# zhongzisha/multi_frame_super_resolution

Measured on AMD Instinct MI355X. Metric: Mpix/s end-to-end (N-frame burst -> x2 SR), higher is better.
Workload: dtype f32

## Files before the change

### include/mfsr.h

```cpp
#ifndef MFSR_H
#define MFSR_H

#include <stddef.h>
#include <stdint.h>

#ifdef __cplusplus
extern "C" {
#endif

#define MFSR_VERSION 100
#define MFSR_MAX_FUSE_GROUP 4
#define MFSR_MAX_BURST_FUSE 16

typedef void* mfsr_stream_t;

typedef struct { float x, y; } mfsr_float2;
typedef struct { float x, y, z; } mfsr_float3;
typedef struct { float x, y, z, w; } mfsr_float4;

typedef struct {
    const void* ptr;
    int32_t pitch;
    int32_t width;
    int32_t height;
// ... 330 lines not shown
    float Dth, Dtr, kDetail, kDenoise, kStretch, kShrink;
    float weightThreshold;
    int32_t applyGamma;
    int32_t fused;
    int32_t pairFrames;
    int32_t asyncFuse;
    int32_t preAlign;
    float preAlignMaxAngle;
    int32_t uploadRing;
    int32_t maskErode;
    int32_t rawPacking;
} mfsr_config;

typedef struct mfsr_burst mfsr_burst;

int mfsr_config_default(mfsr_config* cfg, int width, int height, int frames, int scale, int mono);
size_t mfsr_burst_workspace_bytes(const mfsr_config* cfg);
size_t mfsr_burst_accumulator_bytes(const mfsr_config* cfg);
int mfsr_burst_create(mfsr_burst** out, const mfsr_config* cfg, void* workspace, size_t workspaceBytes);
void mfsr_burst_destroy(mfsr_burst* b);

int mfsr_window_check(const mfsr_config* cfg, int x0, int y0, int w, int h);
int mfsr_burst_set_window(mfsr_burst* b, int x0, int y0, int w, int h);
int mfsr_burst_get_window(const mfsr_burst* b, int* x0, int* y0, int* w, int* h);
int mfsr_burst_set_reference(mfsr_burst* b, const uint16_t* rawRef, mfsr_stream_t stream);
int mfsr_burst_set_reference_rows(mfsr_burst* b, const uint16_t* rawRef, int hrRow0, int hrRow1, mfsr_stream_t stream);
int mfsr_burst_add_frame(mfsr_burst* b, const uint16_t* raw, int isReference, mfsr_float3* imgOut,
                         mfsr_float3* totalWeights, mfsr_stream_t stream);
int mfsr_burst_begin(mfsr_burst* b, mfsr_float3* imgOut, mfsr_float3* totalWeights, mfsr_stream_t stream);
int mfsr_burst_flush(mfsr_burst* b, mfsr_stream_t stream);
int mfsr_burst_hold_fuse(mfsr_burst* b, int enable);
int mfsr_burst_fuse_stats(const mfsr_burst* b, int* burstLaunches, int* groupsFused);
int mfsr_set_burst_fuse(int enable);
int mfsr_burst_finish(mfsr_burst* b, const mfsr_float3* imgOut, const mfsr_float3* totalWeights, mfsr_float3* outImg,
                      uint16_t* out16, mfsr_stream_t stream);
int mfsr_burst_finish_rows(mfsr_burst* b, const mfsr_float3* imgOut, const mfsr_float3* totalWeights,
                           mfsr_float3* outImg, uint16_t* out16, int row0, int rows, mfsr_stream_t stream);
int mfsr_burst_set_reference_host(mfsr_burst* b, const uint16_t* hostRaw, mfsr_stream_t stream);
int mfsr_burst_add_frame_host(mfsr_burst* b, const uint16_t* hostRaw, int isReference, mfsr_float3* imgOut,
                              mfsr_float3* totalWeights, mfsr_stream_t stream);
int mfsr_burst_prefetch_host(mfsr_burst* b, const uint16_t* const* hostRaws, int nFrames, mfsr_stream_t stream);
int mfsr_burst_finish_host(mfsr_burst* b, const mfsr_float3* imgOut, const mfsr_float3* totalWeights, uint16_t* out16Dev,
                           uint16_t* out16Host, mfsr_stream_t stream);
int mfsr_burst_host_sync(mfsr_burst* b);
int mfsr_burst_set_host_row_bytes(mfsr_burst* b, int rowBytes);
int mfsr_burst_field_dims(const mfsr_burst* b, int* flowW, int* flowH, int* maskW, int* maskH);
int mfsr_burst_align_frame(mfsr_burst* b, const uint16_t* raw, int isReference, mfsr_float2* flowOut, int flowPitch,
                           mfsr_float4* maskOut, int maskPitch, mfsr_stream_t stream);
int mfsr_burst_align_frames(mfsr_burst* b, int nFrames, const uint16_t* const* raws, const int* isReference,
                            mfsr_float2* const* flowOut, int flowPitch, mfsr_float4* const* maskOut, int maskPitch,
                            mfsr_stream_t stream);
int mfsr_burst_group_size(const mfsr_config* cfg);
int mfsr_burst_fuse_rows(mfsr_burst* b, int nFrames, const uint16_t* const* raws, const mfsr_float2* const* flows, int flowPitch,
                         const mfsr_float4* const* masks, int maskPitch, mfsr_float3* imgOut, mfsr_float3* totalWeights,
                         int accumulatorsUndefined, int rowBegin, int rowEnd, mfsr_stream_t stream);

typedef struct {
    int32_t rowBegin, rowEnd;
    int32_t flowRow0, flowRows;
    int32_t maskRow0, maskRows;
    int32_t rawRow0, rawRows;
    float maxFlowY;
    int32_t reserved[3];
} mfsr_stripe_plan;
int mfsr_dist_stripe_plan(const mfsr_config* cfg, int worldSize, int rank, int rawHalo, mfsr_stripe_plan* out);
int mfsr_checkFlowBound(const mfsr_float2* flow, int pitch, int width, int rows, float bound, int* flag, mfsr_stream_t stream);
// ... 243 lines not shown
```

### multi_frame_super_resolution_amd/csrc/accumulate_common.hpp

```cpp
#pragma once
#include <type_traits>
#include "common.hpp"

struct Levels3 {
    float white[3], black[3];
};

static inline Levels3 make_levels(mfsr_float3 white, mfsr_float3 black)
{
    Levels3 l;
    l.white[0] = white.x;
    l.white[1] = white.y;
    l.white[2] = white.z;
    l.black[0] = black.x;
    l.black[1] = black.y;
    l.black[2] = black.z;
    return l;
}

template <bool FAST>
__device__ __forceinline__ float tap_weight(int px, int py, float kx, float ky, float kz)
{
    float w = (float)(px * px) * kx + (float)(2 * px * py) * kz + (float)(py * py) * ky;
    if (FAST) {
        const float t = w * -0.72134752044448170368f;
        w = __builtin_amdgcn_exp2f(t);
    } else {
        w = expf(-0.5f * w);
    }
    if (!finitef(w)) w = (px * py == 0) ? 1.0f : 0.0f;
    return w;
}

__device__ __forceinline__ void tap_accumulate(float raw, float w, int color, const float4& cert4, const Levels3& lv,
                                               pix3& pixel, pix3& totalWeight)
// ... 154 lines not shown
        taps(std::false_type{});
    if (sums) {
#pragma unroll
        for (int ch = 0; ch < 3; ch++) {
            const float v = __builtin_fmaf(sumS[ch], wm * invWhite[ch], -(lv.black[ch] * invWhite[ch]) * sumW[ch]);
            if (ch == 0) pixel.x += v;
            if (ch == 1) pixel.y += v;
            if (ch == 2) pixel.z += v;
        }
        totalWeight.x += sumW[0];
        totalWeight.y += sumW[1];
        totalWeight.z += sumW[2];
    }
    (void)outW;
    (void)outH;
}

template <int GEOM, bool FAST, bool SUMS = false>
__device__ __forceinline__ void accumulate_pixel_generic(int x, int y, const uint16_t* __restrict__ dataIn,
                                                         pix3* __restrict__ imgOut, pix3* __restrict__ totalWeights,
                                                         const float4* __restrict__ certaintyMask,
                                                         const mfsr_tex2d& kernelParam, const mfsr_tex2d& shifts,
                                                         const Levels3& lv, int dimX, int dimY, int scale, int strideOut,
                                                         int strideMask, int cfa, int accX0 = 0, int accY0 = 0)
{
    pix3 pixel = row_ptr(imgOut, strideOut, y - accY0)[x - accX0];
    pix3 totalWeight = row_ptr(totalWeights, strideOut, y - accY0)[x - accX0];
    accumulate_pixel_core<GEOM, FAST, SUMS>(x, y, dataIn, certaintyMask, kernelParam, shifts, lv, dimX, dimY, scale, strideMask,
                                      cfa, pixel, totalWeight);
    row_ptr(imgOut, strideOut, y - accY0)[x - accX0] = pixel;
    row_ptr(totalWeights, strideOut, y - accY0)[x - accX0] = totalWeight;
}

struct HrWindow {
    int x0, y0, x1, y1;
    int rel;
};

struct MarginRects {
    int x0[4], y0[4], w[4];
    int start[5];
    int accX0, accY0;
};

inline MarginRects margin_rects(int hrW, int hrH, int M, const HrWindow& w)
{
    const int r[4][4] = {{1, 1, hrW - 1, M}, {1, hrH - M, hrW - 1, hrH - 1}, {1, M, M, hrH - M}, {hrW - M, M, hrW - 1, hrH - M}};
    MarginRects m{};
    m.start[0] = 0;
    for (int i = 0; i < 4; i++) {
        const int x0 = r[i][0] > w.x0 ? r[i][0] : w.x0, x1 = r[i][2] < w.x1 ? r[i][2] : w.x1;
        const int y0 = r[i][1] > w.y0 ? r[i][1] : w.y0, y1 = r[i][3] < w.y1 ? r[i][3] : w.y1;
        const int cw = x1 > x0 ? x1 - x0 : 0, ch = y1 > y0 ? y1 - y0 : 0;
        m.x0[i] = x0;
        m.y0[i] = y0;
        m.w[i] = cw > 0 ? cw : 1;
        m.start[i + 1] = m.start[i] + cw * ch;
    }
    m.accX0 = w.x0;
    m.accY0 = w.y0;
    return m;
}

__device__ __forceinline__ bool margin_rect_pixel(const MarginRects& m, int idx, int& x, int& y)
{
    if (idx >= m.start[4]) return false;
// ... 7 lines not shown
```

### multi_frame_super_resolution_amd/csrc/accumulate_fast.hip

```cpp
#include <cstdlib>

#include "accumulate_common.hpp"
#include <type_traits>

namespace {

template <int CFA>
struct Cfa {
    static constexpr int col(int yp, int xp) { return (CFA >> (2 * ((yp << 1) | xp))) & 3; }
    static constexpr int pos_of(int c)
    {
        int n = 0, p = -1;
        for (int a = 0; a < 4; a++)
            if (((CFA >> (2 * a)) & 3) == c) {
                n++;
                p = a;
            }
        return n == 1 ? p : -1;
    }
    static constexpr int count(int c)
    {
        int n = 0;
        for (int a = 0; a < 4; a++)
            if (((CFA >> (2 * a)) & 3) == c) n++;
// ... 234 lines not shown
        C[jt][2] = selm(mbx, P_(jt, 3), W_(jt, 4));
    }
    strip_pixel_sites<K, CFA>(C, s, mby, nby, mP, mQ, lv, accP, accW);
}

__device__ __forceinline__ void tap_pair_sums(const float (&w)[13], float (&P)[3][4])
{
    auto W_ = [&](int jt, int it) { const int n = jt * 5 + it; return w[n <= 12 ? n : 24 - n]; };
#pragma unroll
    for (int r = 0; r < 3; r++)
#pragma unroll
        for (int i = 0; i < 4; i++) P[r][i] = W_(r, i) + W_(r, i + 1);
}

template <int K, int CFA, int EP = 0, typename MaskF>
__device__ __forceinline__ void strip_pixel(int X, int Y, int sx, int sy, float kx, float ky, float kz,
                                             const uint16_t* __restrict__ raw, int dimX, MaskF mval,
                                             const StripLevels& lv, float* accP, float* accW)
{
    float w[13];
    tap_weights13(kx, ky, kz, w);
    auto rawf = [&](int x0, int y0, float (&s)[3][3]) {
        const uint16_t* r = raw + (size_t)y0 * dimX + x0;
#pragma unroll
        for (int j = 0; j < 3; j++)
#pragma unroll
            for (int i = 0; i < 3; i++) s[j][i] = (float)r[j * dimX + i];
    };
    strip_pixel_w<K, CFA, EP>(X, Y, sx, sy, w, rawf, mval, lv, accP, accW);
}

#define STRIP_MARGIN 16

template <int SCALE, bool WIN = false>
__global__ void __launch_bounds__(256)
    k_accumulateMargin(const uint16_t* __restrict__ raw, pix3* __restrict__ imgOut, pix3* __restrict__ totalWeights,
                       const float4* __restrict__ certaintyMask, mfsr_tex2d kernelParam, mfsr_tex2d shifts, Levels3 glv,
                       int dimX, int dimY, int strideOut, int strideMask, int cfaPacked, int rowBegin, int rowEnd, MarginRects mr)
{
    constexpr int scale = SCALE;
    if constexpr (WIN) {
        int x, y;
        if (!margin_rect_pixel(mr, blockIdx.x * blockDim.x + threadIdx.x, x, y)) return;
        accumulate_pixel_generic<GEOM_FULL, true, true>(x, y, raw, imgOut, totalWeights, certaintyMask, kernelParam, shifts,
                                                                   glv, dimX, dimY, scale, strideOut, strideMask, cfaPacked,
                                                                   mr.accX0, mr.accY0);
        return;
    }
    const int hrW = scale * dimX, hrH = scale * dimY, M = STRIP_MARGIN;
    const int rowLen = hrW - 2;
    const int nTop = (M - 1) * rowLen;
    const int nBot = (M - 1) * rowLen;
    const int sideLen = 2 * (M - 1);
    const int nSide = (hrH - 2 * M) * sideLen;
    const int idx = blockIdx.x * blockDim.x + threadIdx.x;
    int x, y;
    if (idx < nTop) {
        y = 1 + idx / rowLen;
        x = 1 + idx % rowLen;
    } else if (idx < nTop + nBot) {
        const int r = idx - nTop;
        y = hrH - M + r / rowLen;
        x = 1 + r % rowLen;
    } else if (idx < nTop + nBot + nSide) {
        const int r = idx - nTop - nBot;
        y = M + r / sideLen;
        const int c = r % sideLen;
        x = c < M - 1 ? 1 + c : hrW - M + (c - (M - 1));
    } else {
        return;
    }
    if (y < rowBegin || y >= rowEnd) return;
    accumulate_pixel_generic<GEOM_FULL, true, true>(x, y, raw, imgOut, totalWeights, certaintyMask, kernelParam, shifts, glv, dimX,
                                              dimY, scale, strideOut, strideMask, cfaPacked);
}

struct TileFrame {
    const uint16_t* raw;
    const float4* mask;
    mfsr_tex2d shifts;
};
template <int NF>
struct TileFrames {
    TileFrame f[NF];
};

template <int NF, int SCALE, bool WIN = false>
__global__ void __launch_bounds__(64 * NF)
    k_accumulateMarginN(TileFrames<NF> fr, pix3* __restrict__ imgOut, pix3* __restrict__ totalWeights, mfsr_tex2d kernelParam,
                        Levels3 glv, int dimX, int dimY, int strideOut, int strideMask, int cfaPacked, int rowBegin, int rowEnd,
                        MarginRects mr)
{
    constexpr int scale = SCALE;
    __shared__ float sSum[NF][6][64];
    const int hrW = scale * dimX, hrH = scale * dimY, M = STRIP_MARGIN;
    const int rowLen = hrW - 2;
    const int nTop = (M - 1) * rowLen, nBot = (M - 1) * rowLen;
    const int sideLen = 2 * (M - 1);
    const int nSide = (hrH - 2 * M) * sideLen;
    const int lane = threadIdx.x, n = threadIdx.y;
    const int idx = blockIdx.x * 64 + lane;
    int x = 0, y = -1;
    if constexpr (WIN) {
        if (!margin_rect_pixel(mr, idx, x, y)) y = -1;
    } else if (idx < nTop) {
        y = 1 + idx / rowLen;
        x = 1 + idx % rowLen;
    } else if (idx < nTop + nBot) {
        const int r = idx - nTop;
        y = hrH - M + r / rowLen;
        x = 1 + r % rowLen;
    } else if (idx < nTop + nBot + nSide) {
        const int r = idx - nTop - nBot;
        y = M + r / sideLen;
        const int c = r % sideLen;
        x = c < M - 1 ? 1 + c : hrW - M + (c - (M - 1));
    }
    const bool live = y >= rowBegin && y < rowEnd && y >= 0;
    const int ax = WIN ? mr.accX0 : 0, ay = WIN ? mr.accY0 : 0;
    pix3 pixel = {0.0f, 0.0f, 0.0f}, totalWeight = {0.0f, 0.0f, 0.0f};
    if (live) {
        TileFrame F = fr.f[0];
#pragma unroll
        for (int m = 1; m < NF; m++)
            if (n == m) F = fr.f[m];
        accumulate_pixel_core<GEOM_FULL, true, true>(x, y, F.raw, F.mask, kernelParam, F.shifts, glv, dimX, dimY, scale,
                                                                strideMask, cfaPacked, pixel, totalWeight);
    }
    sSum[n][0][lane] = pixel.x;
    sSum[n][1][lane] = pixel.y;
    sSum[n][2][lane] = pixel.z;
    sSum[n][3][lane] = totalWeight.x;
    sSum[n][4][lane] = totalWeight.y;
    sSum[n][5][lane] = totalWeight.z;
    __syncthreads();
    if (n == 0 && live) {
        pix3 a = row_ptr(imgOut, strideOut, y - ay)[x - ax];
        pix3 w = row_ptr(totalWeights, strideOut, y - ay)[x - ax];
#pragma unroll
        for (int m = 0; m < NF; m++) {
            a.x += sSum[m][0][lane];
            a.y += sSum[m][1][lane];
            a.z += sSum[m][2][lane];
            w.x += sSum[m][3][lane];
            w.y += sSum[m][4][lane];
            w.z += sSum[m][5][lane];
        }
        row_ptr(imgOut, strideOut, y - ay)[x - ax] = a;
        row_ptr(totalWeights, strideOut, y - ay)[x - ax] = w;
    }
}

template <int CFA, int FR>
__device__ __forceinline__ void strip_frame(int tx, int Y, int X0, const uint16_t* __restrict__ raw,
// ... 823 lines not shown
                    const int sy = bsy[n] + (int)(int8_t)(sxy[n][1] >> (8 * k));
                    if ((satW >> n) & 1u)
                        strip_pixel_sat<k, CFA>(X0 + k, Y, sx, sy, w, P, rawf, lv, aP, accW);
                    else
                        strip_pixel_w<k, CFA, EP>(X0 + k, Y, sx, sy, w, rawf, mval, lv, aP, accW);
                }
            }
            if (k == 0) asm volatile("s_waitcnt vmcnt(0)" ::: "memory");
            myP[3 * k] += aP[3 * k];
            myP[3 * k + 1] += aP[3 * k + 1];
            myP[3 * k + 2] += aP[3 * k + 2];
        };
        pixel(std::integral_constant<int, 0>{});
        pixel(std::integral_constant<int, 1>{});
        pixel(std::integral_constant<int, 2>{});
        pixel(std::integral_constant<int, 3>{});
        asm volatile("s_waitcnt vmcnt(0)" ::: "memory");
        lane_add12(myW, accW);
        if (safeBits != (1u << NF) - 1u && stripLive) {
#pragma unroll 1
            for (int n = 0; n < NF; n++) {
                if ((safeBits >> n) & 1u) continue;
                const TileFrame F = fr.f[4 * g + n];
                strip_straight<2>(F, myP, myW, X0, Y, hrW, kernelParam, glv, dimX, dimY, strideMask, cfaPacked);
            }
        }
    }
    int Yw = Y;
    asm volatile("" : "+v"(Yw));
    seg.store(&sAcc[0][ly][0], (char*)imgOut + (size_t)Yw * strideOut + segByte, lx);
    seg.store(&sAcc[1][ly][0], (char*)totalWeights + (size_t)Yw * strideOut + segByte, lx);
}

template <int SCALE>
__global__ void __launch_bounds__(256, 4)
    k_accumulateMarginBurst(BurstFrames fr, int nGroups, pix3* __restrict__ imgOut, pix3* __restrict__ totalWeights, mfsr_tex2d kernelParam,
                            Levels3 glv, int dimX, int dimY, int strideOut, int strideMask, int cfaPacked)
{
    constexpr int scale = SCALE, NF = 4;
    __shared__ float sSum[NF][6][64];
    const int hrW = scale * dimX, hrH = scale * dimY, M = STRIP_MARGIN;
    const int rowLen = hrW - 2;
    const int nTop = (M - 1) * rowLen, nBot = (M - 1) * rowLen;
    const int sideLen = 2 * (M - 1);
    const int nSide = (hrH - 2 * M) * sideLen;
    const int lane = threadIdx.x, n = threadIdx.y;
    const int idx = blockIdx.x * 64 + lane;
    int x = 0, y = -1;
    if (idx < nTop) {
        y = 1 + idx / rowLen;
        x = 1 + idx % rowLen;
    } else if (idx < nTop + nBot) {
        const int r = idx - nTop;
        y = hrH - M + r / rowLen;
        x = 1 + r % rowLen;
    } else if (idx < nTop + nBot + nSide) {
        const int r = idx - nTop - nBot;
        y = M + r / sideLen;
        const int c = r % sideLen;
        x = c < M - 1 ? 1 + c : hrW - M + (c - (M - 1));
    }
    const bool live = y >= 0;
    const bool first = n == 0 && live;
    pix3 a = {0.0f, 0.0f, 0.0f}, w = {0.0f, 0.0f, 0.0f};
    if (first) {
        a = row_ptr(imgOut, strideOut, y)[x];
        w = row_ptr(totalWeights, strideOut, y)[x];
    }
#pragma unroll 1
    for (int g = 0; g < nGroups; g++) {
        pix3 pixel = {0.0f, 0.0f, 0.0f}, totalWeight = {0.0f, 0.0f, 0.0f};
        int xg = x, yg = y;
        asm volatile("" : "+v"(xg), "+v"(yg));
        if (live) {
            TileFrame F = fr.f[4 * g];
#pragma unroll
            for (int m = 1; m < NF; m++)
                if (n == m) F = fr.f[4 * g + m];
            accumulate_pixel_core<GEOM_FULL, true, true>(xg, yg, F.raw, F.mask, kernelParam, F.shifts, glv, dimX, dimY, scale,
                                                                    strideMask, cfaPacked, pixel, totalWeight);
        }
        sSum[n][0][lane] = pixel.x;
        sSum[n][1][lane] = pixel.y;
        sSum[n][2][lane] = pixel.z;
        sSum[n][3][lane] = totalWeight.x;
        sSum[n][4][lane] = totalWeight.y;
        sSum[n][5][lane] = totalWeight.z;
        __syncthreads();
        if (first) {
#pragma unroll
            for (int m = 0; m < NF; m++) {
                a.x += sSum[m][0][lane];
                a.y += sSum[m][1][lane];
                a.z += sSum[m][2][lane];
                w.x += sSum[m][3][lane];
                w.y += sSum[m][4][lane];
                w.z += sSum[m][5][lane];
            }
        }
        __syncthreads();
    }
    if (first) {
        row_ptr(imgOut, strideOut, y)[x] = a;
        row_ptr(totalWeights, strideOut, y)[x] = w;
    }
}

template <int K8, int CFA, bool PARITY = false, typename RawF, typename MaskF>
__device__ __forceinline__ void strip_pixel4_w(int X, int Y, int sx, int sy, const float (&w)[13], RawF rawf, MaskF mval,
                                                const StripLevels& lv, float* accP, float* accW)
{
    const int qx = X + sx - 2, qy = Y + sy - 2;
    const int x0 = qx >> 2, y0 = qy >> 2;
// ... 277 lines not shown
                strip_pixel4<5, CFA, true>(X0 + 1, Y, sx[1], sy[1], kxa[1], kya[1], kza[1], raw, dimX, mval, lv, accP, accW);
                strip_pixel4<6, CFA, true>(X0 + 2, Y, sx[2], sy[2], kxa[2], kya[2], kza[2], raw, dimX, mval, lv, accP, accW);
                strip_pixel4<7, CFA, true>(X0 + 3, Y, sx[3], sy[3], kxa[3], kya[3], kza[3], raw, dimX, mval, lv, accP, accW);
            }
        }
    }
    asm volatile("s_waitcnt vmcnt(0)" ::: "memory");
    __syncthreads();
    float* myP = (float*)&sAcc[0][r][0] + (2 * lx + h) * 12;
    float* myW = (float*)&sAcc[1][r][0] + (2 * lx + h) * 12;
    if (safeBits) {
        lane_add12(myP, accP);
        lane_add12(myW, accW);
    }
    if (safeBits != (1u << NF) - 1u && stripLive) {
#pragma unroll 1
        for (int n = 0; n < NF; n++) {
            if ((safeBits >> n) & 1u) continue;
            TileFrame F = fr.f[0];
#pragma unroll
            for (int m = 1; m < NF; m++)
                if (n == m) F = fr.f[m];
            strip_straight<4>(F, myP, myW, X0, Y, hrW, kernelParam, glv, dimX, dimY, strideMask, cfaPacked);
        }
    }
    __syncthreads();
    seg.store(&sAcc[0][r][h * 192], gP, lx);
    seg.store(&sAcc[1][r][h * 192], gW, lx);
}

constexpr int pack_cfa(int c00, int c01, int c10, int c11) { return c00 | (c01 << 2) | (c10 << 4) | (c11 << 6); }

int g_strip_xcd_remap = 1;
int g_strip_use_tile = 1;

bool tile_kernel_ok(mfsr_tex2d kp, mfsr_tex2d sh, int dimX, int dimY)
{
    const int hrW = 2 * dimX, hrH = 2 * dimY;
    return kp.width == sh.width && kp.height == sh.height && kp.width * 4 == hrW && kp.height * 4 == hrH && kp.width >= 4 &&
           (dimX % 4) == 0 && (dimY % 4) == 0 && (uint64_t)dimX * (uint64_t)dimY * 2u < (1ull << 32) && g_strip_use_tile == 1;
}

bool tile_kernel_ok_fr2(mfsr_tex2d kp, mfsr_tex2d sh, int dimX, int dimY)
{
    const int hrW = 2 * dimX, hrH = 2 * dimY;
    return kp.width == sh.width && kp.height == sh.height && kp.width * 2 == hrW && kp.height * 2 == hrH && kp.width >= 4 &&
           (dimX % 4) == 0 && (dimY % 4) == 0 && (uint64_t)dimX * (uint64_t)dimY * 2u < (1ull << 32) && g_strip_use_tile == 1;
}

struct WinLaunch {
    bool on;
    int tileX0, tilesX;
    int x0, x1, y0;
};
WinLaunch win_launch(const HrWindow& w, int hrW, int tileW)
{
    WinLaunch l;
    l.on = w.rel && !(w.x0 == 0 && w.x1 == hrW && w.y0 == 0);
    l.tileX0 = l.on ? w.x0 / tileW : 0;
    l.tilesX = (l.on ? mfsr_cdiv(w.x1, tileW) : mfsr_cdiv(hrW, tileW)) - l.tileX0;
    l.x0 = l.on ? w.x0 : 0;
    l.x1 = l.on ? w.x1 : hrW;
    l.y0 = l.on ? w.y0 : 0;
    return l;
}

// ... 46 lines not shown
}

int zero_rows(mfsr_float3* imgOut, mfsr_float3* totalWeights, int strideOut, int r0, int r1, const WinLaunch& wl, hipStream_t st)
{
    const size_t rowB = (size_t)(wl.x1 - wl.x0) * 12, rows = (size_t)(r1 - r0);
    for (int p2 = 0; p2 < 2; p2++) {
        char* base = (p2 ? (char*)totalWeights : (char*)imgOut) + (size_t)(r0 - wl.y0) * strideOut;
        const hipError_t e = rowB == (size_t)strideOut ? hipMemsetAsync(base, 0, rows * strideOut, st)
                                                       : hipMemset2DAsync(base, strideOut, 0, rowB, rows, st);
        if (e != hipSuccess) return -1;
    }
    return 0;
}

int zero_margin_bands(mfsr_float3* imgOut, mfsr_float3* totalWeights, int hrH, int strideOut, int rowBegin, int rowEnd,
                      const WinLaunch& wl, hipStream_t st)
{
    const int bands[2][2] = {{0, STRIP_MARGIN}, {hrH - STRIP_MARGIN, hrH}};
    for (int i = 0; i < 2; i++) {
        const int r0 = bands[i][0] > rowBegin ? bands[i][0] : rowBegin, r1 = bands[i][1] < rowEnd ? bands[i][1] : rowEnd;
        if (r1 <= r0) continue;
        if (zero_rows(imgOut, totalWeights, strideOut, r0, r1, wl, st) != 0) return -1;
    }
    return 0;
}

long long margin_pixel_count(int hrW, int hrH)
{
    const int M = STRIP_MARGIN;
    return 2LL * (M - 1) * (hrW - 2) + (long long)(hrH - 2 * M) * 2 * (M - 1);
}

template <int SCALE>
void launch_margin_1(hipStream_t st, const uint16_t* raw, const mfsr_float4* mask, mfsr_tex2d shifts, pix3* pI, pix3* pT, mfsr_tex2d kp,
                     Levels3 glv, int dimX, int dimY, int strideOut, int strideMask, int cp, int rowBegin, int rowEnd,
                     const WinLaunch& wl, const MarginRects& mr)
{
    if (!wl.on)
        hipLaunchKernelGGL(k_accumulateMargin<SCALE>, dim3(mfsr_cdiv(margin_pixel_count(SCALE * dimX, SCALE * dimY), 256)), dim3(256), 0,
                           st, raw, pI, pT, (const float4*)mask, kp, shifts, glv, dimX, dimY, strideOut, strideMask, cp, rowBegin, rowEnd,
                           mr);
    else if (mr.start[4] > 0)
        hipLaunchKernelGGL((k_accumulateMargin<SCALE, true>), dim3(mfsr_cdiv(mr.start[4], 256)), dim3(256), 0, st, raw, pI, pT,
                           (const float4*)mask, kp, shifts, glv, dimX, dimY, strideOut, strideMask, cp, rowBegin, rowEnd, mr);
}

template <int NF, int SCALE>
void launch_margin_n(hipStream_t st, const TileFrames<NF>& fr, pix3* pI, pix3* pT, mfsr_tex2d kp, Levels3 glv, int dimX, int dimY,
                     int strideOut, int strideMask, int cp, int rowBegin, int rowEnd, const WinLaunch& wl, const MarginRects& mr)
{
    if (!wl.on)
        hipLaunchKernelGGL((k_accumulateMarginN<NF, SCALE>), dim3(mfsr_cdiv(margin_pixel_count(SCALE * dimX, SCALE * dimY), 64)),
                           dim3(64, NF), 0, st, fr, pI, pT, kp, glv, dimX, dimY, strideOut, strideMask, cp, rowBegin, rowEnd, mr);
    else if (mr.start[4] > 0)
        hipLaunchKernelGGL((k_accumulateMarginN<NF, SCALE, true>), dim3(mfsr_cdiv(mr.start[4], 64)), dim3(64, NF), 0, st, fr, pI, pT, kp,
                           glv, dimX, dimY, strideOut, strideMask, cp, rowBegin, rowEnd, mr);
}

void read_env_once()
{
    static const bool env_read = [] {
        const char* e = getenv("MFSR_STRIP_TILE");
        if (e && e[0] >= '0' && e[0] <= '1') g_strip_use_tile = e[0] - '0';
        const char* x = getenv("MFSR_XCD_REMAP");
        if (x && (x[0] == '0' || x[0] == '1')) g_strip_xcd_remap = x[0] - '0';
        return true;
    }();
    (void)env_read;
}

void make_levels(mfsr_float3 white, mfsr_float3 black, Levels3& glv, StripLevels& lv)
{
    const float wl[3] = {white.x, white.y, white.z}, bl[3] = {black.x, black.y, black.z};
    for (int c = 0; c < 3; c++) {
        glv.white[c] = wl[c];
        glv.black[c] = bl[c];
        lv.black[c] = bl[c];
        lv.invWhite[c] = 1.0f / wl[c];
    }
}

void fill_frames(TileFrame* fr, const uint16_t* const* dataIn, const mfsr_float4* const* certaintyMask, const mfsr_tex2d* shifts, int n)
{
    for (int i = 0; i < n; i++) {
        fr[i].raw = dataIn[i];
        fr[i].mask = (const float4*)certaintyMask[i];
        fr[i].shifts = shifts[i];
    }
}

template <int N>
using int_c = std::integral_constant<int, N>;

template <bool MONO, class F>
int for_cfa(int packed, F f)
{
    constexpr int R = MFSR_RED, G = MFSR_GREEN, B = MFSR_BLUE;
    switch (packed) {
// ... 108 lines not shown
{
    read_env_once();
    if (nFrames < 8 || nFrames > 4 * TILE_BURST_GROUPS || (nFrames & 3)) return 0;
    int cfa[4];
    mfsr_get_cfa_pattern(cfa);
    const int packed2 = pack_cfa(cfa[0], cfa[1], cfa[2], cfa[3]);
    if ((dimX & 1) || ((uintptr_t)imgOut & 15) || ((uintptr_t)totalWeights & 15) || (strideOut & 15)) return 0;
    if (dimX < 2 * STRIP_MARGIN || dimY < 2 * STRIP_MARGIN) return 0;
    for (int n = 0; n < nFrames; n++)
        if (!tile_kernel_ok(kernelParam, shifts[n], dimX, dimY)) return 0;
    Levels3 glv;
    StripLevels lv;
    make_levels(whiteLevel, blackLevel, glv, lv);
    const int hrW = 2 * dimX, hrH = 2 * dimY;
    const WinLaunch wlc = win_launch(HrWindow{0, 0, hrW, hrH, 0}, hrW, 256);
    const int tilesX = wlc.tilesX, tilesY = mfsr_cdiv(hrH, 4);
    const int tilesPerXcd = g_strip_xcd_remap ? mfsr_cdiv(tilesX * tilesY, 8) : 0;
    const dim3 block(64, 4), g1(tilesPerXcd ? 8 * tilesPerXcd : tilesX * tilesY);
    hipStream_t st = mfsr_s(stream);
    pix3* pI = (pix3*)imgOut;
    pix3* pT = (pix3*)totalWeights;
    const int cp = mfsr_cfa_packed();
    BurstFrames fr;
    fill_frames(fr.f, dataIn, certaintyMask, shifts, nFrames);
    for (int n = nFrames; n < 4 * TILE_BURST_GROUPS; n++) fr.f[n] = fr.f[0];
    const int rc = for_cfa<false>(packed2, [&](auto cfaTag) {
        constexpr int CFA = decltype(cfaTag)::value;
        if (fresh && zero_margin_bands(imgOut, totalWeights, hrH, strideOut, 0, hrH, wlc, st) != 0) return -1;
        hipLaunchKernelGGL((k_accumulate2xTileBurst<CFA>), g1, block, 0, st, fr, nFrames / 4, pI, pT, kernelParam, glv, lv, dimX, dimY,
                           strideOut, strideMask, cp, tilesX, tilesY, tilesPerXcd, fresh ? 1 : 0);
        return 1;
    });
    if (rc != 1) return rc;
    hipLaunchKernelGGL((k_accumulateMarginBurst<2>), dim3(mfsr_cdiv(margin_pixel_count(hrW, hrH), 64)), dim3(64, 4), 0, st, fr,
                       nFrames / 4, pI, pT, kernelParam, glv, dimX, dimY, strideOut, strideMask, cp);
    return 1;
}

int mfsr_try_launch_accumulate4x_tile(int nFrames, const uint16_t* const* dataIn, mfsr_float3* imgOut,
                                      mfsr_float3* totalWeights, const mfsr_float4* const* certaintyMask,
                                      mfsr_tex2d kernelParam, const mfsr_tex2d* shifts, mfsr_float3 whiteLevel,
                                      mfsr_float3 blackLevel, int dimX, int dimY, int strideOut, int strideMask,
                                      int fresh, int rowBegin, int rowEnd, int colBegin, int colEnd, int relative,
                                      mfsr_stream_t stream)
{
    read_env_once();
    if (nFrames < 1 || nFrames > 4 || !g_strip_use_tile) return 0;
    int cfa[4];
    mfsr_get_cfa_pattern(cfa);
    for (int i = 0; i < 4; i++)
        if (cfa[i] > MFSR_BLUE) return 0;
    const int packed2 = pack_cfa(cfa[0], cfa[1], cfa[2], cfa[3]);
    const int hrW = 4 * dimX, hrH = 4 * dimY;
    if ((dimX & 1) || (dimY & 1) || ((uintptr_t)imgOut & 15) || ((uintptr_t)totalWeights & 15) || (strideOut & 15)) return 0;
    if (hrW < 4 * STRIP_MARGIN || hrH < 4 * STRIP_MARGIN) return 0;
    for (int n = 0; n < nFrames; n++)
        if (!(kernelParam.width == shifts[n].width && kernelParam.height == shifts[n].height && kernelParam.width * 8 == hrW &&
              kernelParam.height * 8 == hrH && kernelParam.width >= 4))
            return 0;
    Levels3 glv;
    StripLevels lv;
    make_levels(whiteLevel, blackLevel, glv, lv);
    hipStream_t st = mfsr_s(stream);
    pix3* pI = (pix3*)imgOut;
    pix3* pT = (pix3*)totalWeights;
    const int cp = mfsr_cfa_packed();
    const int tileY0 = rowBegin / 2;
    const WinLaunch wlc = win_launch(HrWindow{colBegin, rowBegin, colEnd, rowEnd, relative}, hrW, 512);
    const MarginRects mr = margin_rects(hrW, hrH, STRIP_MARGIN, HrWindow{colBegin, rowBegin, colEnd, rowEnd, relative});
// ... 30 lines not shown
```

Baseline: 25050.

## Accumulate margin pixels via deduplicated LR sample sites and shared per-pixel header

Adds a 'sites' path for x2 margin accumulation. The 5x5 HR tap window maps onto only a few distinct LR raw samples and at most 2x2 certainty cells, so each is loaded once and reused with compile-time carry selection instead of 25 clamped gathers. In the multi-frame kernels, the per-pixel kernel weights, positions and the sums flag are computed once per block into shared memory and shared across the frame lanes. This adds code complexity, a __syncthreads, and a fallback for out-of-range shifts, and it is gated by an env/API switch that is on by default.

Result: faster. 25470 (median of 6 runs) (+1.7%).

```diff
diff --git a/include/mfsr.h b/include/mfsr.h
--- a/include/mfsr.h
+++ b/include/mfsr.h
@@ -386,6 +386,7 @@
 int mfsr_burst_hold_fuse(mfsr_burst* b, int enable);
 int mfsr_burst_fuse_stats(const mfsr_burst* b, int* burstLaunches, int* groupsFused);
 int mfsr_set_burst_fuse(int enable);
+int mfsr_set_margin_sites(int enable);
 int mfsr_burst_finish(mfsr_burst* b, const mfsr_float3* imgOut, const mfsr_float3* totalWeights, mfsr_float3* outImg,
                       uint16_t* out16, mfsr_stream_t stream);
 int mfsr_burst_finish_rows(mfsr_burst* b, const mfsr_float3* imgOut, const mfsr_float3* totalWeights,
diff --git a/multi_frame_super_resolution_amd/csrc/accumulate_common.hpp b/multi_frame_super_resolution_amd/csrc/accumulate_common.hpp
--- a/multi_frame_super_resolution_amd/csrc/accumulate_common.hpp
+++ b/multi_frame_super_resolution_amd/csrc/accumulate_common.hpp
@@ -1,6 +1,8 @@
 #pragma once
 #include <type_traits>
+#include <utility>
 #include "common.hpp"
+#include "margin_sites.hpp"
 
 struct Levels3 {
     float white[3], black[3];
@@ -221,6 +223,192 @@
     row_ptr(totalWeights, strideOut, y - accY0)[x - accX0] = totalWeight;
 }
 
+
+template <int SCALE>
+__device__ __forceinline__ float2 margin_pixel_pos(int x, int y, int dimX, int dimY)
+{
+    return make_float2(((float)x + 0.5f) / (float)(dimX * SCALE), ((float)y + 0.5f) / (float)(dimY * SCALE));
+}
+
+__device__ __forceinline__ bool margin_pixel_sums(const float4& kernel)
+{
+    return kernel.x >= 0.0f && kernel.y >= 0.0f && kernel.z * kernel.z <= kernel.x * kernel.y && kernel.x < 1e30f && kernel.y < 1e30f;
+}
+
+template <int SCALE, bool USE_SUMS, class WF>
+__device__ __forceinline__ void margin_pixel_taps(int x, int y, int sx, int sy, const uint16_t* __restrict__ dataIn,
+                                                  const float4* __restrict__ certaintyMask, const Levels3& lv,
+                                                  const float (&invWhite)[3], float invWm, int dimX, int dimY, int strideMask, int cfa,
+                                                  WF wsym, float (&sumS)[3], float (&sumW)[3], pix3& pixel, pix3& totalWeight)
+{
+    int ppsxA[5], ppxA[5];
+#pragma unroll
+    for (int px = -2; px <= 2; px++) {
+        ppsxA[px + 2] = clampi(floordiv_pos(x + px + sx, SCALE), 0, dimX - 1);
+        ppxA[px + 2] = clampi(floordiv_pos(x + px, SCALE), 0, dimX - 1);
+    }
+#pragma unroll
+    for (int py = -2; py <= 2; py++) {
+        const int ppsy = clampi(floordiv_pos(y + py + sy, SCALE), 0, dimY - 1);
+        const int ppy = clampi(floordiv_pos(y + py, SCALE), 0, dimY - 1);
+        const uint16_t* rawRow = dataIn + (size_t)ppsy * dimX;
+        const float4* maskRow = row_ptr(certaintyMask, strideMask, ppy / 2);
+#pragma unroll
+        for (int px = -2; px <= 2; px++) {
+            const int ppsx = ppsxA[px + 2];
+            const int color = cfa_at(cfa, ppsy, ppsx);
+            const float raw = (float)rawRow[ppsx];
+            const float4 cert4 = maskRow[ppxA[px + 2] / 2];
+            const int n = (py + 2) * 5 + (px + 2);
+            const float w = wsym(n <= 12 ? n : 24 - n);
+            if (USE_SUMS)
+                tap_accumulate_sums(raw, w, color, cert4, invWm, sumS, sumW);
+            else
+                tap_accumulate_fast(raw, w, color, cert4, lv, invWhite, pixel, totalWeight);
+        }
+    }
+}
+
+template <class F, int... I>
+__device__ __forceinline__ void margin_static_for_impl(F&& f, std::integer_sequence<int, I...>)
+{
+    (f(std::integral_constant<int, I>{}), ...);
+}
+template <int N, class F>
+__device__ __forceinline__ void margin_static_for(F&& f)
+{
+    margin_static_for_impl(f, std::make_integer_sequence<int, N>{});
+}
+
+template <int SCALE, class WF>
+__device__ __forceinline__ void margin_pixel_sites(int x, int y, int sx, int sy, const uint16_t* __restrict__ dataIn,
+                                                   const float4* __restrict__ certaintyMask, float invWm, int dimX, int dimY,
+                                                   int strideMask, int cfa, WF wsym, float (&S)[3], float (&W)[3])
+{
+    constexpr int NS = MarginSites<SCALE>::count;
+    int bx, phx, by, phy;
+    margin_axis<SCALE>(x + sx - 2, bx, phx);
+    margin_axis<SCALE>(y + sy - 2, by, phy);
+    int cellX[2], cellY[2], qx, qy;
+    margin_cert_axis<SCALE>(x - 2, dimX, cellX, qx);
+    margin_cert_axis<SCALE>(y - 2, dimY, cellY, qy);
+    float cert[2][2][3];
+#pragma unroll
+    for (int cj = 0; cj < 2; cj++)
+#pragma unroll
+        for (int ci = 0; ci < 2; ci++) {
+            const uint32_t off = (uint32_t)(cellY[cj] * strideMask) + (uint32_t)cellX[ci] * 16u;
+            const float4 c = *(const float4*)((const char*)certaintyMask + off);
+            cert[cj][ci][0] = finitef(c.x) ? c.x : 0.0f;
+            cert[cj][ci][1] = finitef(c.y) ? c.y : 0.0f;
+            cert[cj][ci][2] = finitef(c.z) ? c.z : 0.0f;
+        }
+    uint32_t hotWord = 0;
+#pragma unroll
+    for (int k = 0; k < 4; k++) hotWord |= (1u << (((uint32_t)cfa >> (8 * k)) & 31u)) << (8 * k);
+    int cxA[NS], xsh[NS];
+#pragma unroll
+    for (int i = 0; i < NS; i++) {
+        cxA[i] = margin_site_coord(bx, i, dimX);
+        xsh[i] = (margin_site_cfa_pos(0, cxA[i])) << 3;
+    }
+    float r[NS][NS];
+    uint32_t hot[NS][NS];
+#pragma unroll
+    for (int j = 0; j < NS; j++) {
+        const int ry = margin_site_coord(by, j, dimY);
+        const uint32_t rowOff = (uint32_t)(ry * dimX);
+        const uint32_t rowWord = hotWord >> (margin_site_cfa_pos(ry, 0) << 3);
+#pragma unroll
+        for (int i = 0; i < NS; i++) {
+            r[j][i] = (float)dataIn[rowOff + (uint32_t)cxA[i]] * invWm;
+            hot[j][i] = (rowWord >> xsh[i]) & 0xffu;
+        }
+    }
+    margin_static_for<5>([&](auto jtTag) {
+        constexpr int jt = decltype(jtTag)::value;
+        constexpr int jlo = margin_tap_site_lo<SCALE>(jt), jhi = jlo + 1 < NS ? jlo + 1 : jlo;
+        const bool cy = margin_tap_carry_varies<SCALE>(jt) && margin_tap_carry<SCALE>(phy, jt) != 0;
+        float rRow[NS];
+        uint32_t hotRow[NS];
+#pragma unroll
+        for (int i = 0; i < NS; i++) {
+            rRow[i] = cy ? r[jhi][i] : r[jlo][i];
+            hotRow[i] = cy ? hot[jhi][i] : hot[jlo][i];
+        }
+        const bool my = margin_tap_cell_varies<SCALE>(jt) ? margin_tap_cell<SCALE>(qy, jt) != 0 : jt != 0;
+        float certRow[2][3];
+#pragma unroll
+        for (int ci = 0; ci < 2; ci++)
+#pragma unroll
+            for (int k = 0; k < 3; k++) certRow[ci][k] = my ? cert[1][ci][k] : cert[0][ci][k];
+        margin_static_for<5>([&](auto itTag) {
+            constexpr int it = decltype(itTag)::value;
+            constexpr int ilo = margin_tap_site_lo<SCALE>(it), ihi = ilo + 1 < NS ? ilo + 1 : ilo;
+            const bool cx = margin_tap_carry_varies<SCALE>(it) && margin_tap_carry<SCALE>(phx, it) != 0;
+            const float raw = cx ? rRow[ihi] : rRow[ilo];
+            const uint32_t h = cx ? hotRow[ihi] : hotRow[ilo];
+            uint32_t m[3];
+#pragma unroll
+            for (int c = 0; c < 3; c++) m[c] = (uint32_t)__builtin_amdgcn_sbfe((int)h, c, 1);
+            const bool mx = margin_tap_cell_varies<SCALE>(it) ? margin_tap_cell<SCALE>(qx, it) != 0 : it != 0;
+            const float cR = mx ? certRow[1][0] : certRow[0][0];
+            const float cG = mx ? certRow[1][1] : certRow[0][1];
+            const float cB = mx ? certRow[1][2] : certRow[0][2];
+            const float cc[3] = {cR, cG, cB};
+            const float w = wsym(jt * 5 + it <= 12 ? jt * 5 + it : 24 - (jt * 5 + it));
+#pragma unroll
+            for (int c = 0; c < 3; c++) {
+                const float tc = w * __uint_as_float(m[c] & __float_as_uint(cc[c]));
+                W[c] += tc;
+                S[c] += raw * tc;
+            }
+        });
+    });
+}
+
+template <int SCALE, class WF>
+__device__ __forceinline__ void accumulate_pixel_sites(int x, int y, const uint16_t* __restrict__ dataIn,
+                                                       const float4* __restrict__ certaintyMask, const mfsr_tex2d& shifts,
+                                                       const Levels3& lv, int dimX, int dimY, int strideMask, int cfa, float posX,
+                                                       float posY, bool sums, WF wsym, pix3& pixel, pix3& totalWeight)
+{
+    const float2 shift = tex2<ADDR_CLAMP>(shifts, posX, posY);
+    const int sx = round2i(shift.x * (float)SCALE);
+    const int sy = round2i(shift.y * (float)SCALE);
+    float invWhite[3];
+#pragma unroll
+    for (int ch = 0; ch < 3; ch++) invWhite[ch] = __builtin_amdgcn_rcpf(lv.white[ch]);
+    const float wm = fmaxf(fmaxf(lv.white[0], lv.white[1]), lv.white[2]);
+    const float invWm = __builtin_amdgcn_rcpf(wm);
+    float sumS[3] = {0.0f, 0.0f, 0.0f}, sumW[3] = {0.0f, 0.0f, 0.0f};
+    const bool inRange = (uint32_t)sx + (1u << 30) <= (2u << 30) && (uint32_t)sy + (1u << 30) <= (2u << 30) && finitef(invWm);
+    int xo = x, yo = y, sxo = sx, syo = sy;
+    if (sums && inRange) {
+        margin_pixel_sites<SCALE>(x, y, sx, sy, dataIn, certaintyMask, invWm, dimX, dimY, strideMask, cfa, wsym, sumS, sumW);
+    } else if (sums) {
+        asm volatile("" : "+v"(xo), "+v"(yo), "+v"(sxo), "+v"(syo));
+        margin_pixel_taps<SCALE, true>(xo, yo, sxo, syo, dataIn, certaintyMask, lv, invWhite, invWm, dimX, dimY, strideMask, cfa, wsym, sumS,
+                                       sumW, pixel, totalWeight);
+    } else {
+        asm volatile("" : "+v"(xo), "+v"(yo), "+v"(sxo), "+v"(syo));
+        margin_pixel_taps<SCALE, false>(xo, yo, sxo, syo, dataIn, certaintyMask, lv, invWhite, invWm, dimX, dimY, strideMask, cfa, wsym, sumS,
+                                        sumW, pixel, totalWeight);
+    }
+    if (sums) {
+#pragma unroll
+        for (int ch = 0; ch < 3; ch++) {
+            const float v = __builtin_fmaf(sumS[ch], wm * invWhite[ch], -(lv.black[ch] * invWhite[ch]) * sumW[ch]);
+            if (ch == 0) pixel.x += v;
+            if (ch == 1) pixel.y += v;
+            if (ch == 2) pixel.z += v;
+        }
+        totalWeight.x += sumW[0];
+        totalWeight.y += sumW[1];
+        totalWeight.z += sumW[2];
+    }
+}
+
 struct HrWindow {
     int x0, y0, x1, y1;
     int rel;
diff --git a/multi_frame_super_resolution_amd/csrc/accumulate_fast.hip b/multi_frame_super_resolution_amd/csrc/accumulate_fast.hip
--- a/multi_frame_super_resolution_amd/csrc/accumulate_fast.hip
+++ b/multi_frame_super_resolution_amd/csrc/accumulate_fast.hip
@@ -290,7 +290,31 @@
 
 #define STRIP_MARGIN 16
 
-template <int SCALE, bool WIN = false>
+template <int SCALE, bool SITES>
+__device__ __forceinline__ void margin_pixel_1(int x, int y, const uint16_t* __restrict__ raw, pix3* __restrict__ imgOut,
+                                               pix3* __restrict__ totalWeights, const float4* __restrict__ certaintyMask,
+                                               const mfsr_tex2d& kernelParam, const mfsr_tex2d& shifts, const Levels3& glv, int dimX,
+                                               int dimY, int strideOut, int strideMask, int cfaPacked, int accX0 = 0, int accY0 = 0)
+{
+    if constexpr (SITES) {
+        const float2 pos = margin_pixel_pos<SCALE>(x, y, dimX, dimY);
+        const float4 kernel = tex4<ADDR_CLAMP>(kernelParam, pos.x, pos.y);
+        float wSym[13];
+#pragma unroll
+        for (int n = 0; n < 13; n++) wSym[n] = tap_weight<true>(n % 5 - 2, n / 5 - 2, kernel.x, kernel.y, kernel.z);
+        pix3 pixel = row_ptr(imgOut, strideOut, y - accY0)[x - accX0];
+        pix3 totalWeight = row_ptr(totalWeights, strideOut, y - accY0)[x - accX0];
+        accumulate_pixel_sites<SCALE>(x, y, raw, certaintyMask, shifts, glv, dimX, dimY, strideMask, cfaPacked, pos.x, pos.y,
+                                      margin_pixel_sums(kernel), [&](int n) { return wSym[n]; }, pixel, totalWeight);
+        row_ptr(imgOut, strideOut, y - accY0)[x - accX0] = pixel;
+        row_ptr(totalWeights, strideOut, y - accY0)[x - accX0] = totalWeight;
+    } else {
+        accumulate_pixel_generic<GEOM_FULL, true, true>(x, y, raw, imgOut, totalWeights, certaintyMask, kernelParam, shifts, glv, dimX,
+                                                        dimY, SCALE, strideOut, strideMask, cfaPacked, accX0, accY0);
+    }
+}
+
+template <int SCALE, bool WIN = false, bool SITES = false>
 __global__ void __launch_bounds__(256)
     k_accumulateMargin(const uint16_t* __restrict__ raw, pix3* __restrict__ imgOut, pix3* __restrict__ totalWeights,
                        const float4* __restrict__ certaintyMask, mfsr_tex2d kernelParam, mfsr_tex2d shifts, Levels3 glv,
@@ -300,9 +324,8 @@
     if constexpr (WIN) {
         int x, y;
         if (!margin_rect_pixel(mr, blockIdx.x * blockDim.x + threadIdx.x, x, y)) return;
-        accumulate_pixel_generic<GEOM_FULL, true, true>(x, y, raw, imgOut, totalWeights, certaintyMask, kernelParam, shifts,
-                                                                   glv, dimX, dimY, scale, strideOut, strideMask, cfaPacked,
-                                                                   mr.accX0, mr.accY0);
+        margin_pixel_1<SCALE, SITES>(x, y, raw, imgOut, totalWeights, certaintyMask, kernelParam, shifts, glv, dimX, dimY, strideOut,
+                                     strideMask, cfaPacked, mr.accX0, mr.accY0);
         return;
     }
     const int hrW = scale * dimX, hrH = scale * dimY, M = STRIP_MARGIN;
@@ -329,8 +352,8 @@
         return;
     }
     if (y < rowBegin || y >= rowEnd) return;
-    accumulate_pixel_generic<GEOM_FULL, true, true>(x, y, raw, imgOut, totalWeights, certaintyMask, kernelParam, shifts, glv, dimX,
-                                              dimY, scale, strideOut, strideMask, cfaPacked);
+    margin_pixel_1<SCALE, SITES>(x, y, raw, imgOut, totalWeights, certaintyMask, kernelParam, shifts, glv, dimX, dimY, strideOut,
+                                 strideMask, cfaPacked);
 }
 
 struct TileFrame {
@@ -343,7 +366,29 @@
     TileFrame f[NF];
 };
 
-template <int NF, int SCALE, bool WIN = false>
+struct MarginHeader {
+    float w[13][64];
+    float pos[2][64];
+    int sums[64];
+};
+template <int NF, int SCALE>
+__device__ __forceinline__ void margin_header(MarginHeader& h, bool live, int x, int y, int lane, int n, const mfsr_tex2d& kernelParam,
+                                              int dimX, int dimY)
+{
+    if (live) {
+        const float2 pos = margin_pixel_pos<SCALE>(x, y, dimX, dimY);
+        const float4 kernel = tex4<ADDR_CLAMP>(kernelParam, pos.x, pos.y);
+        if (n == 0) {
+            h.pos[0][lane] = pos.x;
+            h.pos[1][lane] = pos.y;
+        }
+        for (int k = n; k < 13; k += NF) h.w[k][lane] = tap_weight<true>(k % 5 - 2, k / 5 - 2, kernel.x, kernel.y, kernel.z);
+        if (n == 0) h.sums[lane] = margin_pixel_sums(kernel) ? 1 : 0;
+    }
+    __syncthreads();
+}
+
+template <int NF, int SCALE, bool WIN = false, bool SITES = false>
 __global__ void __launch_bounds__(64 * NF)
     k_accumulateMarginN(TileFrames<NF> fr, pix3* __restrict__ imgOut, pix3* __restrict__ totalWeights, mfsr_tex2d kernelParam,
                         Levels3 glv, int dimX, int dimY, int strideOut, int strideMask, int cfaPacked, int rowBegin, int rowEnd,
@@ -356,7 +401,7 @@
     const int nTop = (M - 1) * rowLen, nBot = (M - 1) * rowLen;
     const int sideLen = 2 * (M - 1);
     const int nSide = (hrH - 2 * M) * sideLen;
-    const int lane = threadIdx.x, n = threadIdx.y;
+    const int lane = threadIdx.x, n = SITES ? __builtin_amdgcn_readfirstlane(threadIdx.y) : threadIdx.y;
     const int idx = blockIdx.x * 64 + lane;
     int x = 0, y = -1;
     if constexpr (WIN) {
@@ -377,7 +422,15 @@
     const bool live = y >= rowBegin && y < rowEnd && y >= 0;
     const int ax = WIN ? mr.accX0 : 0, ay = WIN ? mr.accY0 : 0;
     pix3 pixel = {0.0f, 0.0f, 0.0f}, totalWeight = {0.0f, 0.0f, 0.0f};
-    if (live) {
+    if constexpr (SITES) {
+        __shared__ MarginHeader sHdr;
+        margin_header<NF, SCALE>(sHdr, live, x, y, lane, n, kernelParam, dimX, dimY);
+        if (live) {
+            const TileFrame F = fr.f[n];
+            accumulate_pixel_sites<SCALE>(x, y, F.raw, F.mask, F.shifts, glv, dimX, dimY, strideMask, cfaPacked, sHdr.pos[0][lane], sHdr.pos[1][lane],
+                                          sHdr.sums[lane] != 0, [&](int k) { return sHdr.w[k][lane]; }, pixel, totalWeight);
+        }
+    } else if (live) {
         TileFrame F = fr.f[0];
 #pragma unroll
         for (int m = 1; m < NF; m++)
@@ -1267,7 +1320,7 @@
     seg.store(&sAcc[1][ly][0], (char*)totalWeights + (size_t)Yw * strideOut + segByte, lx);
 }
 
-template <int SCALE>
+template <int SCALE, bool SITES = false>
 __global__ void __launch_bounds__(256, 4)
     k_accumulateMarginBurst(BurstFrames fr, int nGroups, pix3* __restrict__ imgOut, pix3* __restrict__ totalWeights, mfsr_tex2d kernelParam,
                             Levels3 glv, int dimX, int dimY, int strideOut, int strideMask, int cfaPacked)
@@ -1279,7 +1332,7 @@
     const int nTop = (M - 1) * rowLen, nBot = (M - 1) * rowLen;
     const int sideLen = 2 * (M - 1);
     const int nSide = (hrH - 2 * M) * sideLen;
-    const int lane = threadIdx.x, n = threadIdx.y;
+    const int lane = threadIdx.x, n = SITES ? __builtin_amdgcn_readfirstlane(threadIdx.y) : threadIdx.y;
     const int idx = blockIdx.x * 64 + lane;
     int x = 0, y = -1;
     if (idx < nTop) {
@@ -1302,18 +1355,31 @@
         a = row_ptr(imgOut, strideOut, y)[x];
         w = row_ptr(totalWeights, strideOut, y)[x];
     }
+    __shared__ MarginHeader sHdr;
+    if constexpr (SITES) margin_header<NF, SCALE>(sHdr, live, x, y, lane, n, kernelParam, dimX, dimY);
 #pragma unroll 1
     for (int g = 0; g < nGroups; g++) {
         pix3 pixel = {0.0f, 0.0f, 0.0f}, totalWeight = {0.0f, 0.0f, 0.0f};
-        int xg = x, yg = y;
-        asm volatile("" : "+v"(xg), "+v"(yg));
-        if (live) {
-            TileFrame F = fr.f[4 * g];
-#pragma unroll
-            for (int m = 1; m < NF; m++)
-                if (n == m) F = fr.f[4 * g + m];
-            accumulate_pixel_core<GEOM_FULL, true, true>(xg, yg, F.raw, F.mask, kernelParam, F.shifts, glv, dimX, dimY, scale,
-                                                                    strideMask, cfaPacked, pixel, totalWeight);
+        if constexpr (SITES) {
+            int xg = x, yg = y;
+            asm volatile("" : "+v"(xg), "+v"(yg));
+            if (live) {
+                const TileFrame F = fr.f[4 * g + n];
+                accumulate_pixel_sites<SCALE>(xg, yg, F.raw, F.mask, F.shifts, glv, dimX, dimY, strideMask, cfaPacked,
+                                              sHdr.pos[0][lane], sHdr.pos[1][lane], sHdr.sums[lane] != 0,
+                                              [&](int k) { return sHdr.w[k][lane]; }, pixel, totalWeight);
+            }
+        } else {
+            int xg = x, yg = y;
+            asm volatile("" : "+v"(xg), "+v"(yg));
+            if (live) {
+                TileFrame F = fr.f[4 * g];
+#pragma unroll
+                for (int m = 1; m < NF; m++)
+                    if (n == m) F = fr.f[4 * g + m];
+                accumulate_pixel_core<GEOM_FULL, true, true>(xg, yg, F.raw, F.mask, kernelParam, F.shifts, glv, dimX, dimY, scale,
+                                                             strideMask, cfaPacked, pixel, totalWeight);
+            }
         }
         sSum[n][0][lane] = pixel.x;
         sSum[n][1][lane] = pixel.y;
@@ -1657,6 +1723,7 @@
 constexpr int pack_cfa(int c00, int c01, int c10, int c11) { return c00 | (c01 << 2) | (c10 << 4) | (c11 << 6); }
 
 int g_strip_xcd_remap = 1;
+int g_margin_sites = 1;
 int g_strip_use_tile = 1;
 
 bool tile_kernel_ok(mfsr_tex2d kp, mfsr_tex2d sh, int dimX, int dimY)
@@ -1769,29 +1836,50 @@
 }
 
 template <int SCALE>
+bool margin_sites_ok(int dimX, int dimY, int strideMask)
+{
+    return SCALE == 2 && g_margin_sites == 1 && (long long)dimX * dimY * 2 < (1LL << 31) &&
+           (long long)strideMask * ((dimY + 1) / 2) < (1LL << 31);
+}
+
+template <int SCALE>
 void launch_margin_1(hipStream_t st, const uint16_t* raw, const mfsr_float4* mask, mfsr_tex2d shifts, pix3* pI, pix3* pT, mfsr_tex2d kp,
                      Levels3 glv, int dimX, int dimY, int strideOut, int strideMask, int cp, int rowBegin, int rowEnd,
                      const WinLaunch& wl, const MarginRects& mr)
 {
-    if (!wl.on)
-        hipLaunchKernelGGL(k_accumulateMargin<SCALE>, dim3(mfsr_cdiv(margin_pixel_count(SCALE * dimX, SCALE * dimY), 256)), dim3(256), 0,
-                           st, raw, pI, pT, (const float4*)mask, kp, shifts, glv, dimX, dimY, strideOut, strideMask, cp, rowBegin, rowEnd,
-                           mr);
-    else if (mr.start[4] > 0)
-        hipLaunchKernelGGL((k_accumulateMargin<SCALE, true>), dim3(mfsr_cdiv(mr.start[4], 256)), dim3(256), 0, st, raw, pI, pT,
-                           (const float4*)mask, kp, shifts, glv, dimX, dimY, strideOut, strideMask, cp, rowBegin, rowEnd, mr);
+    auto launch = [&](auto sites) {
+        constexpr bool SITES = decltype(sites)::value;
+        if (!wl.on)
+            hipLaunchKernelGGL((k_accumulateMargin<SCALE, false, SITES>), dim3(mfsr_cdiv(margin_pixel_count(SCALE * dimX, SCALE * dimY), 256)),
+                               dim3(256), 0, st, raw, pI, pT, (const float4*)mask, kp, shifts, glv, dimX, dimY, strideOut, strideMask, cp,
+                               rowBegin, rowEnd, mr);
+        else if (mr.start[4] > 0)
+            hipLaunchKernelGGL((k_accumulateMargin<SCALE, true, SITES>), dim3(mfsr_cdiv(mr.start[4], 256)), dim3(256), 0, st, raw, pI, pT,
+                               (const float4*)mask, kp, shifts, glv, dimX, dimY, strideOut, strideMask, cp, rowBegin, rowEnd, mr);
+    };
+    if constexpr (SCALE == 2) {
+        if (margin_sites_ok<SCALE>(dimX, dimY, strideMask)) return launch(std::true_type{});
+    }
+    launch(std::false_type{});
 }
 
 template <int NF, int SCALE>
 void launch_margin_n(hipStream_t st, const TileFrames<NF>& fr, pix3* pI, pix3* pT, mfsr_tex2d kp, Levels3 glv, int dimX, int dimY,
                      int strideOut, int strideMask, int cp, int rowBegin, int rowEnd, const WinLaunch& wl, const MarginRects& mr)
 {
-    if (!wl.on)
-        hipLaunchKernelGGL((k_accumulateMarginN<NF, SCALE>), dim3(mfsr_cdiv(margin_pixel_count(SCALE * dimX, SCALE * dimY), 64)),
-                           dim3(64, NF), 0, st, fr, pI, pT, kp, glv, dimX, dimY, strideOut, strideMask, cp, rowBegin, rowEnd, mr);
-    else if (mr.start[4] > 0)
-        hipLaunchKernelGGL((k_accumulateMarginN<NF, SCALE, true>), dim3(mfsr_cdiv(mr.start[4], 64)), dim3(64, NF), 0, st, fr, pI, pT, kp,
-                           glv, dimX, dimY, strideOut, strideMask, cp, rowBegin, rowEnd, mr);
+    auto launch = [&](auto sites) {
+        constexpr bool SITES = decltype(sites)::value;
+        if (!wl.on)
+            hipLaunchKernelGGL((k_accumulateMarginN<NF, SCALE, false, SITES>), dim3(mfsr_cdiv(margin_pixel_count(SCALE * dimX, SCALE * dimY), 64)),
+                               dim3(64, NF), 0, st, fr, pI, pT, kp, glv, dimX, dimY, strideOut, strideMask, cp, rowBegin, rowEnd, mr);
+        else if (mr.start[4] > 0)
+            hipLaunchKernelGGL((k_accumulateMarginN<NF, SCALE, true, SITES>), dim3(mfsr_cdiv(mr.start[4], 64)), dim3(64, NF), 0, st, fr, pI,
+                               pT, kp, glv, dimX, dimY, strideOut, strideMask, cp, rowBegin, rowEnd, mr);
+    };
+    if constexpr (SCALE == 2) {
+        if (margin_sites_ok<SCALE>(dimX, dimY, strideMask)) return launch(std::true_type{});
+    }
+    launch(std::false_type{});
 }
 
 void read_env_once()
@@ -1801,6 +1889,8 @@
         if (e && e[0] >= '0' && e[0] <= '1') g_strip_use_tile = e[0] - '0';
         const char* x = getenv("MFSR_XCD_REMAP");
         if (x && (x[0] == '0' || x[0] == '1')) g_strip_xcd_remap = x[0] - '0';
+        const char* m = getenv("MFSR_MARGIN_SITES");
+        if (m && m[0] == '0') g_margin_sites = 0;
         return true;
     }();
     (void)env_read;
@@ -1975,9 +2065,20 @@
         return 1;
     });
     if (rc != 1) return rc;
-    hipLaunchKernelGGL((k_accumulateMarginBurst<2>), dim3(mfsr_cdiv(margin_pixel_count(hrW, hrH), 64)), dim3(64, 4), 0, st, fr,
-                       nFrames / 4, pI, pT, kernelParam, glv, dimX, dimY, strideOut, strideMask, cp);
+    if (margin_sites_ok<2>(dimX, dimY, strideMask))
+        hipLaunchKernelGGL((k_accumulateMarginBurst<2, true>), dim3(mfsr_cdiv(margin_pixel_count(hrW, hrH), 64)), dim3(64, 4), 0, st, fr,
+                           nFrames / 4, pI, pT, kernelParam, glv, dimX, dimY, strideOut, strideMask, cp);
+    else
+        hipLaunchKernelGGL((k_accumulateMarginBurst<2, false>), dim3(mfsr_cdiv(margin_pixel_count(hrW, hrH), 64)), dim3(64, 4), 0, st, fr,
+                           nFrames / 4, pI, pT, kernelParam, glv, dimX, dimY, strideOut, strideMask, cp);
     return 1;
+}
+
+extern "C" int mfsr_set_margin_sites(int enable)
+{
+    read_env_once();
+    g_margin_sites = enable ? 1 : 0;
+    return MFSR_OK;
 }
 
 int mfsr_try_launch_accumulate4x_tile(int nFrames, const uint16_t* const* dataIn, mfsr_float3* imgOut,
diff --git a/multi_frame_super_resolution_amd/csrc/margin_sites.hpp b/multi_frame_super_resolution_amd/csrc/margin_sites.hpp
--- /dev/null
+++ b/multi_frame_super_resolution_amd/csrc/margin_sites.hpp
@@ -0,0 +1,73 @@
+#pragma once
+
+#if defined(__HIPCC__)
+#define MFSR_SITES_HD __host__ __device__ __forceinline__
+#else
+#define MFSR_SITES_HD inline
+#endif
+
+template <int S>
+MFSR_SITES_HD int margin_floordiv(int a)
+{
+    const int q = a / S;
+    return (a % S < 0) ? q - 1 : q;
+}
+
+MFSR_SITES_HD int margin_clamp(int v, int lo, int hi) { return v < lo ? lo : (v > hi ? hi : v); }
+
+template <int S>
+struct MarginSites {
+    static constexpr int count = (S + 3) / S + 1;
+};
+
+template <int S>
+MFSR_SITES_HD void margin_axis(int u0, int& base, int& phase)
+{
+    base = margin_floordiv<S>(u0);
+    phase = u0 - base * S;
+}
+
+template <int S>
+MFSR_SITES_HD constexpr int margin_tap_site_lo(int it)
+{
+    return it / S;
+}
+template <int S>
+MFSR_SITES_HD constexpr bool margin_tap_carry_varies(int it)
+{
+    return it % S != 0;
+}
+template <int S>
+MFSR_SITES_HD int margin_tap_carry(int phase, int it)
+{
+    return (phase + it % S >= S) ? 1 : 0;
+}
+template <int S>
+MFSR_SITES_HD int margin_tap_site(int phase, int it)
+{
+    return margin_tap_site_lo<S>(it) + margin_tap_carry<S>(phase, it);
+}
+
+MFSR_SITES_HD int margin_site_coord(int base, int site, int dim) { return margin_clamp(base + site, 0, dim - 1); }
+
+MFSR_SITES_HD int margin_site_cfa_pos(int row, int col) { return ((row & 1) << 1) | (col & 1); }
+
+template <int S>
+MFSR_SITES_HD void margin_cert_axis(int x0, int dim, int (&cell)[2], int& phase)
+{
+    const int c = margin_floordiv<2 * S>(x0);
+    phase = x0 - c * 2 * S;
+    cell[0] = margin_clamp(c, 0, (dim - 1) / 2);
+    cell[1] = margin_clamp(c + 1, 0, (dim - 1) / 2);
+}
+
+template <int S>
+MFSR_SITES_HD int margin_tap_cell(int phase, int it)
+{
+    return (phase + it >= 2 * S) ? 1 : 0;
+}
+template <int S>
+MFSR_SITES_HD constexpr bool margin_tap_cell_varies(int it)
+{
+    return it != 0 && it < 2 * S;
+}
```
